# Runki2018/litehandnet

Measured on AMD Instinct MI355X. Metric: images/sec fwd+bwd @256x256 bs64 litehandnet, higher is better.
Workload: dtype f32; 1 GPU; litehandnet variant B (MSRB hourglass litehourglass.py) C=128, 256x256x3 -> 21x64x64, per-GPU batch 64, train-mode BN, fwd + TopdownHeatmapLoss + bwd + fused Adam; global_batch=64, parallelism=dp1

## Files before the change

### litehandnet_amd/csrc/k_conv_dw.hip

```cpp
#include <stdlib.h>
#include "lhn_common.h"

template <int K>
__global__ void __launch_bounds__(256) k_dw_fwd(lhn_view x, const float* __restrict__ w, lhn_view y,
                                                double* __restrict__ stats, int stride, int pad, int dil, lhn_bnfin fin,
                                                int ) {
  extern __shared__ __attribute__((aligned(16))) float smem[];
  const int C = x.C, C4 = C >> 2;
  constexpr int KK = K * K;
  float* Ws = smem;
  f4* red = reinterpret_cast<f4*>(smem + KK * C);
  const int tid = threadIdx.x;
  const int c4 = tid % C4, pl = tid / C4, PL = 256 / C4;
  const int cin = x.coff + 4 * c4, cout = y.coff + 4 * c4;
  const Xf4 xf = lhn_load_xf(x, cin);
  for (int i = tid; i < KK * C; i += 256) {
    const int c = i / KK, t = i - c * KK;
    Ws[t * C + c] = w ? w[i] : 1.f;
  }
  __syncthreads();
  f4 wt[KK];
#pragma unroll
  for (int t = 0; t < KK; ++t) wt[t] = *reinterpret_cast<const f4*>(Ws + t * C + 4 * c4);
  const int rows = y.N * y.H;
// ... 1309 lines not shown
            *reinterpret_cast<f4*>(o) = accx;
          }
        }
      }
    } else {
      if (dx)
        for (int j = 0; j < TH / 2; ++j) {
          const int rr = 2 * j + rpar, hh = th * TH + rr;
          if (wcol < SW && hh < SH && cok) {
            const int centre = ((rr + T::P) * T::WW + colw + T::P) * 8 + c4;
            f4 accx = (f4){0.f, 0.f, 0.f, 0.f};
            for (int a = 0; a < K; ++a)
#pragma unroll
              for (int b = 0; b < K; ++b)
                accx += tdy[centre - ((a * DIL - T::P) * T::WW + (b * DIL - T::P)) * 8] * wl[(a * K + b) * 8 + c4];
            float* o = dx + ((size_t)(n * x.H + pa + ps * hh) * x.W + pb + ps * wcol) * x.cstride + cx;
            if (dx_acc) accx += *reinterpret_cast<const f4*>(o);
            if (bs.add[0]) accx += *reinterpret_cast<const f4*>(bs.add[0] + (o - dx));
            if (bs.add[1]) accx += *reinterpret_cast<const f4*>(bs.add[1] + (o - dx));
            *reinterpret_cast<f4*>(o) = accx;
          }
        }
      for (int a = 0; a < K; ++a) {
        f4 ar[K];
#pragma unroll
        for (int b = 0; b < K; ++b) ar[b] = (f4){0.f, 0.f, 0.f, 0.f};
        for (int j = 0; j < TH / 2; ++j) {
          const int rr = 2 * j + rpar, hh = th * TH + rr;
          if (wcol < SW && hh < SH) {
            const int centre = ((rr + T::P) * T::WW + colw + T::P) * 8 + c4;
            const f4 dyc = tdy[centre];
#pragma unroll
            for (int b = 0; b < K; ++b) ar[b] += dyc * tx[centre + ((a * DIL - T::P) * T::WW + (b * DIL - T::P)) * 8];
          }
        }
#pragma unroll
        for (int b = 0; b < K; ++b) {
          f4 v = ar[b];
#pragma unroll
          for (int o = 8; o < 64; o <<= 1) {
            v.x += __shfl_xor(v.x, o, 64);
            v.y += __shfl_xor(v.y, o, 64);
            v.z += __shfl_xor(v.z, o, 64);
            v.w += __shfl_xor(v.w, o, 64);
          }
          if ((tid & 63) < 8) red[(tid >> 6) * 8 + c4 + 32 * b] = v;
        }
        __syncthreads();
        if (tid < 8 * K) {
          const int b = tid >> 3, cc = tid & 7;
          dws[(a * K + b) * 8 + cc] += red[cc + 32 * b] + red[8 + cc + 32 * b] + red[16 + cc + 32 * b] + red[24 + cc + 32 * b];
        }
        __syncthreads();
      }
    }
  }
  if (BNS) {
    double* st = bs.sums + (size_t)((bid / cgroups) % LHN_STAT_REPLICAS) * 2 * bs.C + bs.coff + cg * 32;
    lhn_block_stat_atomics(sdu, sdux, 8, red, st, st + bs.C);
  }
  float* dwr = dw + (size_t)((bid / cgroups) % nrep) * rep_stride;
  if (REGACC) {
#pragma unroll
    for (int k = 0; k < KK; ++k)
#pragma unroll
      for (int o = 8; o < 64; o <<= 1) {
        accw[k].x += __shfl_xor(accw[k].x, o, 64);
        accw[k].y += __shfl_xor(accw[k].y, o, 64);
        accw[k].z += __shfl_xor(accw[k].z, o, 64);
        accw[k].w += __shfl_xor(accw[k].w, o, 64);
      }
    __syncthreads();
    if ((tid & 63) < 8)
#pragma unroll
      for (int k = 0; k < KK; ++k) tdy[(k * 4 + (tid >> 6)) * 8 + c4] = accw[k];
    __syncthreads();
    if (tid < KK * 8) {
      const int k = tid >> 3, cc = tid & 7;
      const f4 sacc = tdy[(k * 4 + 0) * 8 + cc] + tdy[(k * 4 + 1) * 8 + cc] + tdy[(k * 4 + 2) * 8 + cc] + tdy[(k * 4 + 3) * 8 + cc];
      const int cb = cg * 32 + 4 * cc;
      if (cc < cvalid) {
        atomicAdd(dwr + (cb + 0) * KK + k, sacc.x);
        atomicAdd(dwr + (cb + 1) * KK + k, sacc.y);
        atomicAdd(dwr + (cb + 2) * KK + k, sacc.z);
        atomicAdd(dwr + (cb + 3) * KK + k, sacc.w);
      }
    }
  } else {
    __syncthreads();
    for (int i = tid; i < KK * 8; i += 256) {
      const int k = i >> 3, cb = cg * 32 + 4 * (i & 7);
      const f4 v = dws[i];
      if ((i & 7) >= cvalid) continue;
      atomicAdd(dwr + (cb + 0) * KK + k, v.x);
      atomicAdd(dwr + (cb + 1) * KK + k, v.y);
      atomicAdd(dwr + (cb + 2) * KK + k, v.z);
      atomicAdd(dwr + (cb + 3) * KK + k, v.w);
    }
  }
}

template <int DIL, bool BNS = false>
__global__ void __launch_bounds__(256, (BNS || DIL > 1) ? 2 : 3) k_dw3_bwd_rows(lhn_view x, const float* __restrict__ w, lhn_view y, lhn_gradview gy,
                                                         float* __restrict__ dx, int dx_acc, float* __restrict__ dw, int nstrips,
                                                         int nchunks, int CH, int cgroups, int nrep, int64_t rep_stride, int ps,
                                                         DwBnSum bs, lhn_bnbwdsrc fs) {
  constexpr int P = DIL, R = 2 * P + 2, WW = 32 + 2 * P, KK = 9;
  extern __shared__ __attribute__((aligned(16))) float smem[];
  f4* tdy = reinterpret_cast<f4*>(smem);
  f4* tx = tdy + R * WW * 8;
  f4* wl = tx + R * WW * 8;
  f4* cst = wl + KK * 8;
  f4* tmi = cst + KK * 8;
  f4* traw = tmi + 16;
  const int tid = threadIdx.x, c4 = tid & 7, pl = tid >> 3;
  const int ntile = y.N * ps * ps * nchunks * nstrips * cgroups;
  const int cg = blockIdx.x % cgroups;
  const int cvalid = min(8, (x.C - cg * 32) >> 2);
  const bool cok = c4 < cvalid;
  const int c4e = cok ? c4 : 0;
  const int cx = x.coff + cg * 32 + 4 * c4e, cy = y.coff + cg * 32 + 4 * c4e;
  const bool edge = tid < 16 * P;
  const int ecol = (pl < P) ? pl : 32 + pl;
  const f4 z = (f4){0.f, 0.f, 0.f, 0.f}, one = (f4){1.f, 1.f, 1.f, 1.f};
  if (tid < KK * 8) {
    const int k = tid >> 3, cc = cg * 32 + 4 * min(tid & 7, cvalid - 1);
    wl[tid] = (f4){w[(cc + 0) * KK + k], w[(cc + 1) * KK + k], w[(cc + 2) * KK + k], w[(cc + 3) * KK + k]};
  } else if (tid < 2 * KK * 8) {
    const int i = tid - KK * 8, kind = i >> 3, ca = cg * 32 + 4 * min(i & 7, cvalid - 1), j = kind % 3;
    const float* tab = kind < 3 ? x.table : kind < 6 ? y.table : gy.coef;
    const int cs = kind < 3 ? x.cstride : y.cstride, co = kind < 3 ? x.coff : y.coff;
    if (kind < 6 || !fs.sums) cst[i] = tab ? *reinterpret_cast<const f4*>(tab + j * cs + co + ca) : ((kind < 6 ? j != 1 : j == 0) ? one : z);
  } else if (BNS && tid < 2 * KK * 8 + 16) {
    const int i = tid - 2 * KK * 8, kind = i >> 3, cc = i & 7;
    tmi[i] = *reinterpret_cast<const f4*>(bs.save + kind * bs.C + bs.coff + cg * 32 + 4 * cc);
  }
  f4 accw[KK];
#pragma unroll
  for (int k = 0; k < KK; ++k) accw[k] = z;
  f4 sdu = z, sdux = z;
  struct Item {
    int n, pa, pb, SH, SW, wb, h0, nrows;
  };
  auto decode = [&](int t) __attribute__((always_inline)) {
    Item it;
    int r = t / cgroups;
    const int st = r % nstrips;
    r /= nstrips;
    const int ch = r % nchunks;
    r /= nchunks;
    const int par = r % (ps * ps);
    it.n = r / (ps * ps);
    it.pa = par / ps;
    it.pb = par % ps;
    it.SH = (x.H - it.pa + ps - 1) / ps;
    it.SW = (x.W - it.pb + ps - 1) / ps;
    it.wb = st * 32;
    it.h0 = ch * CH;
    it.nrows = max(0, min(CH, it.SH - it.h0));
    return it;
  };
  f4 mx = z, my = z, mz = z, mp = z, ex = z, ey = z, ez = z, ep = z;
  bool okm = false, oke = false;
  auto issue = [&](const Item& it, int hr) __attribute__((always_inline)) {
    const bool rok = hr >= 0 && hr < it.SH && cok;
    const int ih = it.pa + ps * hr;
    const int cm = it.wb + pl, ce = it.wb - P + ecol;
    okm = rok && cm < it.SW;
    oke = rok && edge && ce >= 0 && ce < it.SW;
    mx = my = mz = mp = ex = ey = ez = ep = z;
    if (okm) {
      const size_t pix = (size_t)(it.n * x.H + ih) * x.W + it.pb + ps * cm;
      mx = *reinterpret_cast<const f4*>(x.data + pix * x.cstride + cx);
      my = *reinterpret_cast<const f4*>(y.data + pix * y.cstride + cy);
      mz = *reinterpret_cast<const f4*>(gy.dz + pix * y.cstride + cy);
      if (gy.dpool) mp = lhn_dpool_sum(gy, y, it.n, ih, it.pb + ps * cm, cy);
    }
    if (oke) {
      const size_t pix = (size_t)(it.n * x.H + ih) * x.W + it.pb + ps * ce;
      ex = *reinterpret_cast<const f4*>(x.data + pix * x.cstride + cx);
      ey = *reinterpret_cast<const f4*>(y.data + pix * y.cstride + cy);
      ez = *reinterpret_cast<const f4*>(gy.dz + pix * y.cstride + cy);
      if (gy.dpool) ep = lhn_dpool_sum(gy, y, it.n, ih, it.pb + ps * ce, cy);
    }
  };
  auto put = [&](int s, int col, bool ok, f4 rx, f4 ry, f4 rz, f4 rp, f4 xg, f4 yg) __attribute__((always_inline)) {
    const f4 xsc = cst[c4], xsh = cst[8 + c4], xsl = cst[16 + c4];
    const f4 ysc = cst[24 + c4], ysh = cst[32 + c4], ysl = cst[40 + c4];
    const f4 gA = cst[48 + c4], gB = cst[56 + c4], gC = cst[64 + c4];
    const f4 ux = rx * xsc + xsh;
    const f4 vx = (f4){lhn_lrelu(ux.x, xsl.x), lhn_lrelu(ux.y, xsl.y), lhn_lrelu(ux.z, xsl.z), lhn_lrelu(ux.w, xsl.w)} * xg;
    const f4 e = rz * yg + rp;
    const f4 u = ry * ysc + ysh;
    const f4 dl = (f4){u.x > 0.f ? 1.f : ysl.x, u.y > 0.f ? 1.f : ysl.y, u.z > 0.f ? 1.f : ysl.z, u.w > 0.f ? 1.f : ysl.w};
    const f4 vy = gA * (e * dl) + gB * ry + gC;
    tx[(s * WW + col) * 8 + c4] = ok ? vx : z;
    tdy[(s * WW + col) * 8 + c4] = ok ? vy : z;
    if (BNS && col >= P && col < 32 + P) traw[(s * 32 + col - P) * 8 + c4] = rx;
  };
  int t = blockIdx.x;
  if (t < ntile) {
    const Item nx = decode(t);
    issue(nx, nx.h0 - P);
  }
  if (fs.sums) {
    float* cfA = reinterpret_cast<float*>(cst + 6 * 8);
    if (tid >= 4 * cvalid && tid < 32) cfA[tid] = cfA[32 + tid] = cfA[64 + tid] = 0.f;
    double* raw = reinterpret_cast<double*>(tdy);
    const int nc = 4 * cvalid;
    const LhnBwdPre pre = lhn_bn_bwd_pre(fs, cg * 32, nc);
    lhn_bn_bwd_fold_raw(fs.sums, fs.stat_channels, cg * 32, nc, raw);
    __syncthreads();
    if (tid < nc)
      lhn_bn_bwd_coef_put(lhn_bn_bwd_coef_raw(raw, nc, lhn_fin_groups(y.C), tid, pre, fs.count), fs, const_cast<float*>(gy.coef), y.cstride,
                          y.coff, cg * 32 + tid, cfA, 32, tid, (int)blockIdx.x < cgroups);
  }
#pragma unroll 1
  for (; t < ntile; t += gridDim.x) {
    const Item it = decode(t);
    const f4 xg = x.gate ? *reinterpret_cast<const f4*>(x.gate + (size_t)it.n * x.cstride + cx) : one;
    const f4 yg = y.gate ? *reinterpret_cast<const f4*>(y.gate + (size_t)it.n * y.cstride + cy) : one;
    const int wcol = it.wb + pl, nload = it.nrows + 2 * P;
    const bool ocol = wcol < it.SW;
    __syncthreads();
#pragma unroll 1
    for (int q = 0; q < nload; ++q) {
      const bool orow = q >= 2 * P;
      const int hh = it.h0 + max(q - 2 * P, 0);
      float* o = dx + ((size_t)(it.n * x.H + it.pa + ps * hh) * x.W + it.pb + ps * wcol) * x.cstride + cx;
      const bool st = orow && dx && cok && ocol;
      const int s = q % R;
      put(s, pl + P, okm, mx, my, mz, mp, xg, yg);
      if (edge) put(s, ecol, oke, ex, ey, ez, ep, xg, yg);
      if (q + 1 < nload) issue(it, it.h0 - P + q + 1);
      else if (t + (int)gridDim.x < ntile) {
        const Item nx = decode(t + gridDim.x);
        issue(nx, nx.h0 - P);
      }
      __syncthreads();
      if (!orow || !ocol) continue;
      int sr[3];
#pragma unroll
      for (int a = 0; a < 3; ++a) sr[a] = (q - 2 * P + a * DIL) % R;
      const int centre = (sr[1] * WW + pl + P) * 8 + c4;
      const f4 dyc = tdy[centre];
      f4 accx = z;
#pragma unroll
      for (int a = 0; a < 3; ++a) {
#pragma unroll
        for (int b = 0; b < 3; ++b) {
          accx += tdy[(sr[2 - a] * WW + pl + 2 * P - b * DIL) * 8 + c4] * wl[(a * 3 + b) * 8 + c4];
          accw[a * 3 + b] += dyc * tx[(sr[a] * WW + pl + b * DIL) * 8 + c4];
        }
      }
      if (BNS) {
        const f4 raw = traw[(sr[1] * 32 + pl) * 8 + c4];
        const f4 xsc = cst[c4], xsh = cst[8 + c4], xsl = cst[16 + c4];
        const f4 u = raw * xsc + xsh;
        const f4 du = accx * (f4){u.x > 0.f ? 1.f : xsl.x, u.y > 0.f ? 1.f : xsl.y, u.z > 0.f ? 1.f : xsl.z, u.w > 0.f ? 1.f : xsl.w};
        sdu += du;
        sdux += du * ((raw - tmi[c4]) * tmi[8 + c4]);
      }
      if (st) {
        if (dx_acc) accx += *reinterpret_cast<const f4*>(o);
        if (bs.add[0]) accx += *reinterpret_cast<const f4*>(bs.add[0] + (o - dx));
        if (bs.add[1]) accx += *reinterpret_cast<const f4*>(bs.add[1] + (o - dx));
        *reinterpret_cast<f4*>(o) = accx;
      }
    }
  }
  f4* red = tdy;
  if (BNS) {
    double* sts = bs.sums + (size_t)((blockIdx.x / cgroups) % LHN_STAT_REPLICAS) * 2 * bs.C + bs.coff + cg * 32;
    lhn_block_stat_atomics(sdu, sdux, 8, red, sts, sts + bs.C);
  }
  float* dwr = dw + (size_t)((blockIdx.x / cgroups) % nrep) * rep_stride;
#pragma unroll
  for (int k = 0; k < KK; ++k)
#pragma unroll
    for (int o = 8; o < 64; o <<= 1) {
      accw[k].x += __shfl_xor(accw[k].x, o, 64);
      accw[k].y += __shfl_xor(accw[k].y, o, 64);
      accw[k].z += __shfl_xor(accw[k].z, o, 64);
      accw[k].w += __shfl_xor(accw[k].w, o, 64);
    }
  __syncthreads();
  if ((tid & 63) < 8)
#pragma unroll
    for (int k = 0; k < KK; ++k) red[(k * 4 + (tid >> 6)) * 8 + c4] = accw[k];
  __syncthreads();
  if (tid < KK * 8) {
    const int k = tid >> 3, cc = tid & 7;
    const f4 sacc = red[(k * 4 + 0) * 8 + cc] + red[(k * 4 + 1) * 8 + cc] + red[(k * 4 + 2) * 8 + cc] + red[(k * 4 + 3) * 8 + cc];
    const int cb = cg * 32 + 4 * cc;
    if (cc < cvalid) {
      atomicAdd(dwr + (cb + 0) * KK + k, sacc.x);
      atomicAdd(dwr + (cb + 1) * KK + k, sacc.y);
      atomicAdd(dwr + (cb + 2) * KK + k, sacc.z);
      atomicAdd(dwr + (cb + 3) * KK + k, sacc.w);
    }
  }
}

static int dw3_xchunk(int grid, int cgroups) {
  static int on = -1;
  if (on < 0) {
    const char* e = getenv("LHN_XCD_ORDER");
    on = (e && e[0] == '1') ? 1 : 0;
  }
  return (on && grid % (8 * cgroups) == 0) ? grid / 8 : 0;
}
static int dw3_grid(int ntile, int cgroups, int per_cu) {
  int g = lhn_num_cus() * per_cu;
  g -= g % cgroups;
  if (g > ntile) g = ntile;
  if (g < cgroups) g = cgroups;
  return g;
}

template <int K, int DIL, int NS = 1>
static void launch_dwk_fwd(const lhn_view* x, const float* w, const lhn_view* y, double* stats, lhn_bnfin fin, hipStream_t s, int ps = 1,
                           const DwExtra* exp = nullptr) {
  DwExtra ex;
  if (exp) ex = *exp; else { ex.n = 0; ex.sum_out = nullptr; }
  constexpr int TH = 8, TW = 32, P = DIL * (K - 1) / 2;
  const int cg = (x->C + 31) / 32;
  const int sh = (y->H + ps - 1) / ps, sw = (y->W + ps - 1) / ps;
  const int th = (sh + TH - 1) / TH, tw = (sw + TW - 1) / TW, ntile = y->N * ps * ps * th * tw * cg;
  const size_t lds = (size_t)((TH + 2 * P) * (TW + 2 * P) * 8 + 512 + K * K * 8) * 16;
  const int per_cu = lds > 80 * 1024 ? 1 : (lds > 52 * 1024 ? 2 : 3);
  static LhnKernelCfg cfg;
  (void)lhn_kernel_cfg(cfg, &k_dwk_fwd_lds<K, DIL, NS>, lds, 4, nullptr);
  const int grid = dw3_grid(ntile, cg, per_cu * 2);
  hipLaunchKernelGGL((k_dwk_fwd_lds<K, DIL, NS>), dim3(grid), dim3(256), lds, s, *x, w, *y, stats, th, tw, cg, fin, ps, ex, dw3_xchunk(grid, cg));
}
template <int K, int DIL, bool BNS = false>
static void launch_dwk_bwd(const lhn_view* x, const float* w, const lhn_view* y, const lhn_gradview* gy, float* dx, int dx_acc,
                           float* dw, int nrep, int64_t rep_stride, hipStream_t s, int ps = 1, const DwBnSum* bsp = nullptr) {
  constexpr int TH = 8, TW = 16, P = DIL * (K - 1) / 2;
  DwBnSum bs;
  if (bsp) bs = *bsp; else { bs.sums = nullptr; bs.save = nullptr; bs.C = bs.coff = 0; bs.add[0] = bs.add[1] = nullptr; }
  const int cg = (x->C + 31) / 32;
  const int sh = (x->H + ps - 1) / ps, sw = (x->W + ps - 1) / ps;
  const int th = (sh + TH - 1) / TH, tw = (sw + TW - 1) / TW, ntile = x->N * ps * ps * th * tw * cg;
  const size_t lds = (size_t)((TH + 2 * P) * (TW + 2 * P) * 16 + 256 + 2 * K * K * 8 + (BNS ? TH * TW * 8 + 16 : 0)) * 16;
  static LhnKernelCfg cfg;
  (void)lhn_kernel_cfg(cfg, &k_dwk_bwd_lds<K, DIL, BNS>, lds, 4, nullptr);
  const int grid = dw3_grid(ntile, cg, 4);
  hipLaunchKernelGGL((k_dwk_bwd_lds<K, DIL, BNS>), dim3(grid), dim3(256), lds, s, *x, w, *y, *gy, dx, dx_acc, dw, th, tw,
                     cg, nrep, rep_stride, ps, bs, dw3_xchunk(grid, cg));
}
template <int DIL, bool BNS = false>
static void launch_dw3_bwd_rows(const lhn_view* x, const float* w, const lhn_view* y, const lhn_gradview* gy, float* dx, int dx_acc,
                                float* dw, int nrep, int64_t rep_stride, hipStream_t s, int ps = 1, const DwBnSum* bsp = nullptr,
                                const lhn_bnbwdsrc* fsp = nullptr) {
  constexpr int P = DIL, R = 2 * P + 2, WW = 32 + 2 * P;
  DwBnSum bs;
  if (bsp) bs = *bsp; else { bs.sums = nullptr; bs.save = nullptr; bs.C = bs.coff = 0; bs.add[0] = bs.add[1] = nullptr; }
  lhn_bnbwdsrc fs;
  if (fsp) fs = *fsp; else memset(&fs, 0, sizeof(fs));
  static_assert(R * WW * 8 * 16 >= 2 * LHN_FIN_THREADS * 8, "dy ring holds the replica fold's partials");
  const int cg = (x->C + 31) / 32;
  const int sh = (x->H + ps - 1) / ps, sw = (x->W + ps - 1) / ps;
  const int nstrips = (sw + 31) / 32;
  const size_t lds = (size_t)(2 * R * WW * 8 + 2 * 9 * 8 + 16 + (BNS ? R * 32 * 8 : 0)) * 16;
  static LhnKernelCfg cfg;
  int per_cu = 1;
  (void)lhn_kernel_cfg(cfg, &k_dw3_bwd_rows<DIL, BNS>, lds, 8, &per_cu);
  const int base = x->N * ps * ps * nstrips * cg;
  int nch = (lhn_num_cus() * per_cu + base - 1) / base;
  nch = std::max(1, std::min(nch, (sh + 7) / 8));
  const int CH = (sh + nch - 1) / nch;
  nch = (sh + CH - 1) / CH;
  const int ntile = base * nch;
  const int grid = dw3_grid(ntile, cg, per_cu);
  hipLaunchKernelGGL((k_dw3_bwd_rows<DIL, BNS>), dim3(grid), dim3(256), lds, s, *x, w, *y, *gy, dx, dx_acc, dw, nstrips, nch, CH, cg,
                     nrep, rep_stride, ps, bs, fs);
}
static bool lhn_dw_bwd_v1() {
  static int v = -1;
  if (v < 0) {
    const char* e = getenv("LHN_DW_BWD_V1");
    v = (e && e[0] == '1') ? 1 : 0;
  }
  return v == 1;
}


struct DwS2 {
  static constexpr int TH = 4, TW = 16, XH = 2 * TH + 1, XW = 2 * TW + 1, XPIX = XH * XW, DH = TH + 1, DW = TW + 1, DPIX = DH * DW;
};

__global__ void __launch_bounds__(256) k_dws2_fwd_lds(lhn_view x, const float* __restrict__ w, lhn_view y, double* __restrict__ stats,
                                                      int tiles_h, int tiles_w, int cgroups, lhn_bnfin fin) {
  using T = DwS2;
  extern __shared__ __attribute__((aligned(16))) float smem[];
  f4* tx = reinterpret_cast<f4*>(smem);
  f4* red = tx + T::XPIX * 8;
  f4* wl = red + 512;
  const int tid = threadIdx.x, c4 = tid & 7, pl = tid >> 3;
  const int ntile = y.N * tiles_h * tiles_w * cgroups;
  const int cg = blockIdx.x % cgroups;
  const int cvalid = min(8, (x.C - cg * 32) >> 2);
  const bool cok = c4 < cvalid;
  const int c4e = cok ? c4 : 0;
  const int cin = x.coff + cg * 32 + 4 * c4e, cout = y.coff + cg * 32 + 4 * c4e;
  for (int i = tid; i < 72; i += 256) {
    const int k = i >> 3, cc = cg * 32 + 4 * min(i & 7, cvalid - 1);
    wl[i] = (f4){w[(cc + 0) * 9 + k], w[(cc + 1) * 9 + k], w[(cc + 2) * 9 + k], w[(cc + 3) * 9 + k]};
  }
  const Xf4 xf = lhn_load_xf(x, cin);
  double sd[4] = {0, 0, 0, 0}, qd[4] = {0, 0, 0, 0};
  constexpr int NIT = (T::XPIX + 31) / 32;
  for (int t = blockIdx.x; t < ntile; t += gridDim.x) {
    int r = t / cgroups;
    const int tw = r % tiles_w;
    r /= tiles_w;
    const int th = r % tiles_h, n = r / tiles_h;
    const int h0 = 2 * th * T::TH - 1, w0 = 2 * tw * T::TW - 1;
    const f4 gate = x.gate ? *reinterpret_cast<const f4*>(x.gate + (size_t)n * x.cstride + cin) : (f4){1.f, 1.f, 1.f, 1.f};
    const float* xin = x.data + (size_t)n * x.H * x.W * x.cstride + cin;
    f4 raw[NIT];
#pragma unroll
    for (int it = 0; it < NIT; ++it) {
      const int i = min(pl + 32 * it, T::XPIX - 1);
      const int ph = i / T::XW, pw = i - ph * T::XW;
      const int ih = min(max(h0 + ph, 0), x.H - 1), iw = min(max(w0 + pw, 0), x.W - 1);
      raw[it] = *reinterpret_cast<const f4*>(xin + ((size_t)ih * x.W + iw) * x.cstride);
    }
    __syncthreads();
#pragma unroll
    for (int it = 0; it < NIT; ++it) {
      const int i = pl + 32 * it;
      if (i < T::XPIX) {
        const int ph = i / T::XW, pw = i - ph * T::XW;
        const int ih = h0 + ph, iw = w0 + pw;
        const bool inb = ih >= 0 && ih < x.H && iw >= 0 && iw < x.W;
        tx[i * 8 + c4] = inb ? lhn_apply_xf(raw[it], xf) * gate : (f4){0.f, 0.f, 0.f, 0.f};
      }
    }
    __syncthreads();
    f4 s = (f4){0.f, 0.f, 0.f, 0.f}, q = s, kk = s;
    int cnt = 0;
#pragma unroll
    for (int j = 0; j < 2; ++j) {
      const int o = pl + 32 * j, oh = o / T::TW, ow = o - oh * T::TW;
      const int ho = th * T::TH + oh, wo = tw * T::TW + ow;
      if (cok && ho < y.H && wo < y.W) {
        f4 acc = (f4){0.f, 0.f, 0.f, 0.f};
#pragma unroll
        for (int a = 0; a < 3; ++a)
#pragma unroll
          for (int b = 0; b < 3; ++b) acc += tx[((2 * oh + a) * T::XW + 2 * ow + b) * 8 + c4] * wl[(a * 3 + b) * 8 + c4];
        *reinterpret_cast<f4*>(y.data + ((size_t)(n * y.H + ho) * y.W + wo) * y.cstride + cout) = acc;
        if (cnt == 0) kk = acc;
        const f4 d = acc - kk;
        s += d;
        q += d * d;
        ++cnt;
      }
    }
    lhn_unshift4(sd, qd, s, q, kk, cnt);
  }
  if (stats) {
    const int C = x.C;
    double* st = stats + (size_t)((blockIdx.x / cgroups) % LHN_STAT_REPLICAS) * 2 * C + cg * 32;
    lhn_block_stat_atomics_d(sd, qd, 8, reinterpret_cast<double*>(red), st, st + C, cvalid);
    if (fin.counter && lhn_last_block(fin.counter)) lhn_bn_finalize_block(fin, stats);
  }
}

__global__ void __launch_bounds__(256, 2) k_dws2_bwd_lds(lhn_view x, const float* __restrict__ w, lhn_view y, lhn_gradview gy,
                                                      float* __restrict__ dx, int dx_acc, float* __restrict__ dw, int tiles_h,
                                                      int tiles_w, int cgroups, int nrep, int64_t rep_stride) {
  using T = DwS2;
  extern __shared__ __attribute__((aligned(16))) float smem[];
  f4* tx = reinterpret_cast<f4*>(smem);
  f4* tdy = tx + T::XPIX * 8;
  f4* wl = tdy + T::DPIX * 8;
  const int tid = threadIdx.x, c4 = tid & 7, pl = tid >> 3;
  const int ntile = y.N * tiles_h * tiles_w * cgroups;
  const int cg = blockIdx.x % cgroups;
  const int cvalid = min(8, (x.C - cg * 32) >> 2);
  const bool cok = c4 < cvalid;
  const int c4e = cok ? c4 : 0;
  const int cx = x.coff + cg * 32 + 4 * c4e, cy = y.coff + cg * 32 + 4 * c4e;
  const Xf4 xxf = lhn_load_xf(x, cx), yxf = lhn_load_xf(y, cy);
  const Gr4 ygr = lhn_load_coef(gy, y.cstride, cy);
  for (int i = tid; i < 72; i += 256) {
    const int k = i >> 3, cc = cg * 32 + 4 * min(i & 7, cvalid - 1);
    wl[i] = (f4){w[(cc + 0) * 9 + k], w[(cc + 1) * 9 + k], w[(cc + 2) * 9 + k], w[(cc + 3) * 9 + k]};
  }
  f4 accw[9];
#pragma unroll
  for (int k = 0; k < 9; ++k) accw[k] = (f4){0.f, 0.f, 0.f, 0.f};
  constexpr int NITX = (T::XPIX + 31) / 32, NITD = (T::DPIX + 31) / 32;
  for (int t = blockIdx.x; t < ntile; t += gridDim.x) {
    int r = t / cgroups;
    const int tw = r % tiles_w;
    r /= tiles_w;
    const int th = r % tiles_h, n = r / tiles_h;
    const int h0 = 2 * th * T::TH - 1, w0 = 2 * tw * T::TW - 1;
    const int oh0 = th * T::TH, ow0 = tw * T::TW;
    const f4 xgate = x.gate ? *reinterpret_cast<const f4*>(x.gate + (size_t)n * x.cstride + cx) : (f4){1.f, 1.f, 1.f, 1.f};
    f4 rx[NITX], ry[NITD], rz[NITD];
#pragma unroll
    for (int it = 0; it < NITX; ++it) {
      const int i = min(pl + 32 * it, T::XPIX - 1);
      const int ph = i / T::XW, pw = i - ph * T::XW;
      const int ih = min(max(h0 + ph, 0), x.H - 1), iw = min(max(w0 + pw, 0), x.W - 1);
      rx[it] = *reinterpret_cast<const f4*>(x.data + ((size_t)(n * x.H + ih) * x.W + iw) * x.cstride + cx);
    }
#pragma unroll
    for (int it = 0; it < NITD; ++it) {
      const int i = min(pl + 32 * it, T::DPIX - 1);
      const int ph = i / T::DW, pw = i - ph * T::DW;
      const int ho = min(oh0 + ph, y.H - 1), wo = min(ow0 + pw, y.W - 1);
      const size_t off = ((size_t)(n * y.H + ho) * y.W + wo) * y.cstride + cy;
      ry[it] = *reinterpret_cast<const f4*>(y.data + off);
      rz[it] = *reinterpret_cast<const f4*>(gy.dz + off);
    }
    __syncthreads();
#pragma unroll
    for (int it = 0; it < NITX; ++it) {
      const int i = pl + 32 * it;
      if (i < T::XPIX) {
        const int ph = i / T::XW, pw = i - ph * T::XW;
        const int ih = h0 + ph, iw = w0 + pw;
        const bool inb = ih >= 0 && ih < x.H && iw >= 0 && iw < x.W;
        tx[i * 8 + c4] = inb ? lhn_apply_xf(rx[it], xxf) * xgate : (f4){0.f, 0.f, 0.f, 0.f};
      }
    }
#pragma unroll
    for (int it = 0; it < NITD; ++it) {
      const int i = pl + 32 * it;
      if (i < T::DPIX) {
        const int ph = i / T::DW, pw = i - ph * T::DW;
        const int ho = oh0 + ph, wo = ow0 + pw;
        f4 d = (f4){0.f, 0.f, 0.f, 0.f};
        if (ho < y.H && wo < y.W) {
          const f4 du = lhn_grad_du(y, gy, yxf, ry[it], rz[it], n, ho, wo, cy);
          d = ygr.A * du + ygr.B * ry[it] + ygr.Cc;
        }
        tdy[i * 8 + c4] = d;
      }
    }
    __syncthreads();
#pragma unroll
    for (int j = 0; j < 2; ++j) {
      const int o = pl + 32 * j, oh = o / T::TW, ow = o - oh * T::TW;
      const f4 dyc = tdy[(oh * T::DW + ow) * 8 + c4];
#pragma unroll
      for (int a = 0; a < 3; ++a)
#pragma unroll
        for (int b = 0; b < 3; ++b) accw[a * 3 + b] += dyc * tx[((2 * oh + a) * T::XW + 2 * ow + b) * 8 + c4];
    }
    if (dx && cok) {
      const int c = pl, iw = 2 * ow0 + c;
      const int nb = (c & 1) ? 2 : 1;
      const int bA = (c & 1) ? 0 : 1, colA = (c & 1) ? (c + 1) >> 1 : c >> 1, colB = (c - 1) >> 1;
      if (iw < x.W) {
#pragma unroll
        for (int rr = 0; rr < 2 * T::TH; ++rr) {
          const int ih = 2 * oh0 + rr;
          if (ih < x.H) {
            f4 accx = (f4){0.f, 0.f, 0.f, 0.f};
            if ((rr & 1) == 0) {
              const f4* drow = tdy + ((rr >> 1) * T::DW) * 8 + c4;
              accx += drow[colA * 8] * wl[(3 + bA) * 8 + c4];
              if (nb == 2) accx += drow[colB * 8] * wl[(3 + 2) * 8 + c4];
            } else {
              const f4* d0 = tdy + (((rr + 1) >> 1) * T::DW) * 8 + c4;
              const f4* d2 = tdy + (((rr - 1) >> 1) * T::DW) * 8 + c4;
              accx += d0[colA * 8] * wl[(0 + bA) * 8 + c4] + d2[colA * 8] * wl[(6 + bA) * 8 + c4];
              if (nb == 2) accx += d0[colB * 8] * wl[(0 + 2) * 8 + c4] + d2[colB * 8] * wl[(6 + 2) * 8 + c4];
            }
            float* o = dx + ((size_t)(n * x.H + ih) * x.W + iw) * x.cstride + cx;
            if (dx_acc) accx += *reinterpret_cast<const f4*>(o);
            *reinterpret_cast<f4*>(o) = accx;
          }
        }
      }
    }
  }
  float* dwr = dw + (size_t)((blockIdx.x / cgroups) % nrep) * rep_stride;
#pragma unroll
  for (int k = 0; k < 9; ++k)
#pragma unroll
    for (int o = 8; o < 64; o <<= 1) {
      accw[k].x += __shfl_xor(accw[k].x, o, 64);
      accw[k].y += __shfl_xor(accw[k].y, o, 64);
      accw[k].z += __shfl_xor(accw[k].z, o, 64);
      accw[k].w += __shfl_xor(accw[k].w, o, 64);
    }
  __syncthreads();
  if ((tid & 63) < 8)
#pragma unroll
    for (int k = 0; k < 9; ++k) tdy[(k * 4 + (tid >> 6)) * 8 + c4] = accw[k];
  __syncthreads();
  if (tid < 72) {
    const int k = tid >> 3, cc = tid & 7;
    const f4 sacc = tdy[(k * 4 + 0) * 8 + cc] + tdy[(k * 4 + 1) * 8 + cc] + tdy[(k * 4 + 2) * 8 + cc] + tdy[(k * 4 + 3) * 8 + cc];
    const int cb = cg * 32 + 4 * cc;
    if (cc < cvalid) {
      atomicAdd(dwr + (cb + 0) * 9 + k, sacc.x);
      atomicAdd(dwr + (cb + 1) * 9 + k, sacc.y);
      atomicAdd(dwr + (cb + 2) * 9 + k, sacc.z);
      atomicAdd(dwr + (cb + 3) * 9 + k, sacc.w);
    }
  }
}

static int dws2_fwd(const lhn_view* x, const float* w, const lhn_view* y, double* stats, lhn_bnfin fin, hipStream_t s) {
  using T = DwS2;
  const int cg = (x->C + 31) / 32;
  const int th = (y->H + T::TH - 1) / T::TH, tw = (y->W + T::TW - 1) / T::TW, ntile = y->N * th * tw * cg;
  size_t lds = (size_t)(T::XPIX * 8 + 512 + 72) * 16;
  static LhnKernelCfg cfg;
  if (!lhn_kernel_cfg(cfg, &k_dws2_fwd_lds, lds, 4, nullptr)) return 0;
  hipLaunchKernelGGL(k_dws2_fwd_lds, dim3(dw3_grid(ntile, cg, 6)), dim3(256), lds, s, *x, w, *y, stats, th, tw, cg, fin);
  return 1;
}
static int dws2_bwd(const lhn_view* x, const float* w, const lhn_view* y, const lhn_gradview* gy, float* dx, int dx_acc, float* dw,
                    int nrep, int64_t rep_stride, hipStream_t s) {
  using T = DwS2;
  const int cg = (x->C + 31) / 32;
  const int th = (y->H + T::TH - 1) / T::TH, tw = (y->W + T::TW - 1) / T::TW, ntile = y->N * th * tw * cg;
  const size_t lds = (size_t)((T::XPIX + T::DPIX) * 8 + 72) * 16;
  static LhnKernelCfg cfg;
  if (!lhn_kernel_cfg(cfg, &k_dws2_bwd_lds, lds, 4, nullptr)) return 0;
  hipLaunchKernelGGL(k_dws2_bwd_lds, dim3(dw3_grid(ntile, cg, 4)), dim3(256), lds, s, *x, w, *y, *gy, dx, dx_acc, dw, th, tw, cg, nrep, rep_stride);
  return 1;
}

int lhn_dwk_fwd_lds(const lhn_view* x, const float* w, const lhn_view* y, double* stats, int k, int dil, lhn_bnfin fin,
                    hipStream_t s, const DwExtra* ex) {
  if (ex && ex->n > 0) {
    if (k == 3 && dil == 1) launch_dwk_fwd<3, 1, 2>(x, w, y, stats, fin, s, 1, ex);
    else if (k == 3 && dil == 2 && y->W >= 16) launch_dwk_fwd<3, 1, 2>(x, w, y, stats, fin, s, 2, ex);
    else return 0;
    return 1;
  }
  if (k == 3 && dil == 1) launch_dwk_fwd<3, 1>(x, w, y, stats, fin, s, 1, ex);
  else if (k == 3 && dil == 2 && y->W >= 16) launch_dwk_fwd<3, 1>(x, w, y, stats, fin, s, 2, ex);
  else if (k == 3 && dil == 2) launch_dwk_fwd<3, 2>(x, w, y, stats, fin, s, 1, ex);
  else if (k == 7 && dil == 1) launch_dwk_fwd<7, 1>(x, w, y, stats, fin, s, 1, ex);
  else return 0;
  return 1;
}
int lhn_dwk_bwd_lds(const lhn_view* x, const float* w, const lhn_view* y, const lhn_gradview* gy, float* dx, int dx_acc,
                    float* dw, int k, int dil, int nrep, int64_t rep_stride, hipStream_t s, const DwBnSum* bs,
                    const lhn_bnbwdsrc* fs) {
  if (fs && (lhn_dw_bwd_v1() || k != 3)) return 0;
  if (bs && bs->sums) {
    if (!(k == 3 && dil == 1 && dx && !dx_acc)) return 0;
    if (lhn_dw_bwd_v1()) launch_dwk_bwd<3, 1, true>(x, w, y, gy, dx, dx_acc, dw, nrep, rep_stride, s, 1, bs);
    else launch_dw3_bwd_rows<1, true>(x, w, y, gy, dx, dx_acc, dw, nrep, rep_stride, s, 1, bs, fs);
    return 1;
  }
  const bool v1 = lhn_dw_bwd_v1();
  if (k == 3 && dil == 1) {
    if (v1) launch_dwk_bwd<3, 1>(x, w, y, gy, dx, dx_acc, dw, nrep, rep_stride, s, 1, bs);
    else launch_dw3_bwd_rows<1>(x, w, y, gy, dx, dx_acc, dw, nrep, rep_stride, s, 1, bs, fs);
  } else if (k == 3 && dil == 2 && x->W >= 16) {
    if (v1) launch_dwk_bwd<3, 1>(x, w, y, gy, dx, dx_acc, dw, nrep, rep_stride, s, 2, bs);
    else launch_dw3_bwd_rows<1>(x, w, y, gy, dx, dx_acc, dw, nrep, rep_stride, s, 2, bs, fs);
  } else if (k == 3 && dil == 2) {
    if (v1) launch_dwk_bwd<3, 2>(x, w, y, gy, dx, dx_acc, dw, nrep, rep_stride, s, 1, bs);
    else launch_dw3_bwd_rows<2>(x, w, y, gy, dx, dx_acc, dw, nrep, rep_stride, s, 1, bs, fs);
  } else if (k == 7 && dil == 1) launch_dwk_bwd<7, 1>(x, w, y, gy, dx, dx_acc, dw, nrep, rep_stride, s, 1, bs);
  else return 0;
  return 1;
}

static int dw_fwd_extra(const lhn_view* x, const float* w, const lhn_view* y, double* stats, int k, int stride, int pad, int dil,
                        lhn_bnfin fin, const lhn_view* extra, const float* coef, const lhn_view* so, hipStream_t s) {
  if (!(stride == 1 && pad == dil * (k - 1) / 2 && x->C % 4 == 0 && y->W >= 8)) return 0;
  if (!lhn_no_pend(x) || !lhn_no_pend(extra)) return 0;
  DwExtra ex;
  ex.v = *extra;
  ex.coef[0] = coef[0];
  ex.coef[1] = coef[1];
  ex.n = 1;
  ex.sum_out = so ? so->data : nullptr;
  ex.so_cstride = so ? so->cstride : 0;
  ex.so_coff = so ? so->coff : 0;
  return lhn_dwk_fwd_lds(x, w, y, stats, k, dil, fin, s, &ex);
}

static int dw_bwd_addends(const lhn_view* x, const float* w, const lhn_view* y, const lhn_gradview* gy, float* dx, int dx_acc, float* dw,
                          int k, int dil, int nrep, int64_t rep_stride, const float* a0, const float* a1, hipStream_t s) {
  DwBnSum bs;
  bs.sums = nullptr;
  bs.save = nullptr;
  bs.C = bs.coff = 0;
  bs.add[0] = a0;
  bs.add[1] = a1;
  return lhn_dwk_bwd_lds(x, w, y, gy, dx, dx_acc, dw, k, dil, nrep, rep_stride, s, &bs);
}

static int dw_bwd_fin(const lhn_view* x, const float* w, const lhn_view* y, const lhn_gradview* gy, float* dx, int dx_acc, float* dw, int k,
                      int dil, int nrep, int64_t rep_stride, const lhn_bnsum* bns, const float* a0, const float* a1, const lhn_bnbwdsrc* fin,
                      hipStream_t s) {
  DwBnSum bs;
  bs.sums = bns ? bns->sums : nullptr;
  bs.save = bns ? bns->save : nullptr;
  bs.C = bns ? bns->C : 0;
  bs.coff = bns ? bns->coff : 0;
  bs.add[0] = a0;
  bs.add[1] = a1;
  return lhn_dwk_bwd_lds(x, w, y, gy, dx, dx_acc, dw, k, dil, nrep, rep_stride, s, &bs, fin);
}

static int dw_bwd_fused(const lhn_view* x, const float* w, const lhn_view* y, const lhn_gradview* gy, float* dx, float* dw, int k,
                        int dil, int nrep, int64_t rep_stride, double* bn_sums, const float* bn_save, int bn_C, int bn_coff, hipStream_t s) {
  DwBnSum bs;
  bs.sums = bn_sums;
  bs.save = bn_save;
  bs.C = bn_C;
  bs.coff = bn_coff;
  bs.add[0] = bs.add[1] = nullptr;
  return lhn_dwk_bwd_lds(x, w, y, gy, dx, 0, dw, k, dil, nrep, rep_stride, s, &bs);
}
```

Measured before the change: 8994 images/s.

## Add 8x8 spatial-tile depthwise 3x3 backward kernel for small feature maps

Adds a new depthwise 3x3 backward kernel that works on 8x8 output tiles with a one-pixel halo in LDS. It prefetches the next tile's x, y and dy into registers while computing the current one, and accumulates the weight gradient per block with shuffle reduction and atomics. A dispatcher sends small feature maps (up to 32x32, with few total tiles) to this kernel instead of the row-strip kernel. The aim is to give small layers more parallelism than row strips can. The cost is more halo loads per tile and more dw atomics.

Measured after the change: 9037 images/s (median of 6 runs). Within noise of the previous version (+0.5%).

```diff
diff --git a/litehandnet_amd/csrc/k_conv_dw.hip b/litehandnet_amd/csrc/k_conv_dw.hip
--- a/litehandnet_amd/csrc/k_conv_dw.hip
+++ b/litehandnet_amd/csrc/k_conv_dw.hip
@@ -1635,6 +1635,206 @@
   }
 }
 
+template <bool BNS = false>
+__global__ void __launch_bounds__(256, 2) k_dw3_bwd_tile(lhn_view x, const float* __restrict__ w, lhn_view y, lhn_gradview gy,
+                                                         float* __restrict__ dx, int dx_acc, float* __restrict__ dw, int tiles_h,
+                                                         int tiles_w, int cgroups, int nrep, int64_t rep_stride, int ps, DwBnSum bs,
+                                                         lhn_bnbwdsrc fs) {
+  constexpr int TH = 8, TW = 8, WW = TW + 2, PIX = (TH + 2) * WW, KK = 9, NIT = (PIX + 31) / 32;
+  constexpr int RP = 32 / TW, NJ = TH / RP;
+  static_assert(2 * PIX * 8 * 16 >= 2 * LHN_FIN_THREADS * 8, "the two tiles hold the replica fold's partials");
+  extern __shared__ __attribute__((aligned(16))) float smem[];
+  f4* tdy = reinterpret_cast<f4*>(smem);
+  f4* tx = tdy + PIX * 8;
+  f4* wl = tx + PIX * 8;
+  f4* cst = wl + KK * 8;
+  f4* tmi = cst + KK * 8;
+  f4* traw = tmi + 16;
+  const int tid = threadIdx.x, c4 = tid & 7, pl = tid >> 3;
+  const int colw = pl % TW, rpar = pl / TW;
+  const int ntile = y.N * ps * ps * tiles_h * tiles_w * cgroups;
+  const int cg = blockIdx.x % cgroups;
+  const int cvalid = min(8, (x.C - cg * 32) >> 2);
+  const bool cok = c4 < cvalid;
+  const int c4e = cok ? c4 : 0;
+  const int cx = x.coff + cg * 32 + 4 * c4e, cy = y.coff + cg * 32 + 4 * c4e;
+  const f4 z = (f4){0.f, 0.f, 0.f, 0.f}, one = (f4){1.f, 1.f, 1.f, 1.f};
+  f4 accw[KK];
+#pragma unroll
+  for (int k = 0; k < KK; ++k) accw[k] = z;
+  f4 sdu = z, sdux = z;
+  struct Item {
+    int n, pa, pb, SH, SW, th, tw;
+  };
+  auto decode = [&](int t) __attribute__((always_inline)) {
+    Item it;
+    int r = t / cgroups;
+    it.tw = r % tiles_w;
+    r /= tiles_w;
+    it.th = r % tiles_h;
+    r /= tiles_h;
+    const int par = r % (ps * ps);
+    it.n = r / (ps * ps);
+    it.pa = par / ps;
+    it.pb = par % ps;
+    it.SH = (x.H - it.pa + ps - 1) / ps;
+    it.SW = (x.W - it.pb + ps - 1) / ps;
+    return it;
+  };
+  f4 rx[NIT], ry[NIT], rz[NIT], rp[NIT], xg = one, yg = one;
+#pragma unroll
+  for (int q = 0; q < NIT; ++q) rp[q] = z;
+  auto issue = [&](const Item& it) __attribute__((always_inline)) {
+    const int h0 = it.th * TH - 1, w0 = it.tw * TW - 1;
+    const size_t img = (size_t)it.n * x.H * x.W;
+    const float* xb = x.data + img * x.cstride;
+    const float* yb = y.data + img * y.cstride;
+    const float* zb = gy.dz + img * y.cstride;
+#pragma unroll
+    for (int q = 0; q < NIT; ++q) {
+      const int i = min(pl + 32 * q, PIX - 1);
+      const int ph = i / WW, pw = i - ph * WW;
+      const int ih = min(it.pa + ps * min(max(h0 + ph, 0), max(it.SH - 1, 0)), x.H - 1);
+      const int iw = min(it.pb + ps * min(max(w0 + pw, 0), max(it.SW - 1, 0)), x.W - 1);
+      const unsigned pix = (unsigned)(ih * x.W + iw);
+      rx[q] = *reinterpret_cast<const f4*>(xb + (pix * (unsigned)x.cstride + (unsigned)cx));
+      ry[q] = *reinterpret_cast<const f4*>(yb + (pix * (unsigned)y.cstride + (unsigned)cy));
+      rz[q] = *reinterpret_cast<const f4*>(zb + (pix * (unsigned)y.cstride + (unsigned)cy));
+      if (gy.dpool) rp[q] = lhn_dpool_sum(gy, y, it.n, ih, iw, cy);
+    }
+    if (x.gate) xg = *reinterpret_cast<const f4*>(x.gate + (size_t)it.n * x.cstride + cx);
+    if (y.gate) yg = *reinterpret_cast<const f4*>(y.gate + (size_t)it.n * y.cstride + cy);
+  };
+  auto commit = [&](const Item& it) __attribute__((always_inline)) {
+    const int h0 = it.th * TH - 1, w0 = it.tw * TW - 1;
+    const f4 xsc = cst[c4], xsh = cst[8 + c4], xsl = cst[16 + c4];
+    const f4 ysc = cst[24 + c4], ysh = cst[32 + c4], ysl = cst[40 + c4];
+    const f4 gA = cst[48 + c4], gB = cst[56 + c4], gC = cst[64 + c4];
+#pragma unroll
+    for (int q = 0; q < NIT; ++q) {
+      const int i = pl + 32 * q;
+      if (i < PIX) {
+        const int ph = i / WW, pw = i - ph * WW;
+        const int hh = h0 + ph, ww = w0 + pw;
+        const bool inb = hh >= 0 && hh < it.SH && ww >= 0 && ww < it.SW;
+        const f4 ux = rx[q] * xsc + xsh;
+        const f4 vx = (f4){lhn_lrelu(ux.x, xsl.x), lhn_lrelu(ux.y, xsl.y), lhn_lrelu(ux.z, xsl.z), lhn_lrelu(ux.w, xsl.w)} * xg;
+        const f4 e = rz[q] * yg + rp[q];
+        const f4 u = ry[q] * ysc + ysh;
+        const f4 dl = (f4){u.x > 0.f ? 1.f : ysl.x, u.y > 0.f ? 1.f : ysl.y, u.z > 0.f ? 1.f : ysl.z, u.w > 0.f ? 1.f : ysl.w};
+        const f4 vy = gA * (e * dl) + gB * ry[q] + gC;
+        tx[i * 8 + c4] = inb ? vx : z;
+        tdy[i * 8 + c4] = inb ? vy : z;
+        if (BNS && ph >= 1 && ph <= TH && pw >= 1 && pw <= TW) traw[((ph - 1) * TW + pw - 1) * 8 + c4] = rx[q];
+      }
+    }
+  };
+  int t = blockIdx.x;
+  if (t < ntile) issue(decode(t));
+  if (tid < KK * 8) {
+    const int k = tid >> 3, cc = cg * 32 + 4 * min(tid & 7, cvalid - 1);
+    wl[tid] = (f4){w[(cc + 0) * KK + k], w[(cc + 1) * KK + k], w[(cc + 2) * KK + k], w[(cc + 3) * KK + k]};
+  } else if (tid < 2 * KK * 8) {
+    const int i = tid - KK * 8, kind = i >> 3, ca = cg * 32 + 4 * min(i & 7, cvalid - 1), j = kind % 3;
+    const float* tab = kind < 3 ? x.table : kind < 6 ? y.table : gy.coef;
+    const int cs = kind < 3 ? x.cstride : y.cstride, co = kind < 3 ? x.coff : y.coff;
+    if (kind < 6 || !fs.sums) cst[i] = tab ? *reinterpret_cast<const f4*>(tab + j * cs + co + ca) : ((kind < 6 ? j != 1 : j == 0) ? one : z);
+  } else if (BNS && tid < 2 * KK * 8 + 16) {
+    const int i = tid - 2 * KK * 8, kind = i >> 3, cc = i & 7;
+    tmi[i] = *reinterpret_cast<const f4*>(bs.save + kind * bs.C + bs.coff + cg * 32 + 4 * cc);
+  }
+  if (fs.sums) {
+    float* cfA = reinterpret_cast<float*>(cst + 6 * 8);
+    if (tid >= 4 * cvalid && tid < 32) cfA[tid] = cfA[32 + tid] = cfA[64 + tid] = 0.f;
+    double* raw = reinterpret_cast<double*>(tdy);
+    const int nc = 4 * cvalid;
+    const LhnBwdPre pre = lhn_bn_bwd_pre(fs, cg * 32, nc);
+    lhn_bn_bwd_fold_raw(fs.sums, fs.stat_channels, cg * 32, nc, raw);
+    __syncthreads();
+    if (tid < nc)
+      lhn_bn_bwd_coef_put(lhn_bn_bwd_coef_raw(raw, nc, lhn_fin_groups(y.C), tid, pre, fs.count), fs, const_cast<float*>(gy.coef), y.cstride,
+                          y.coff, cg * 32 + tid, cfA, 32, tid, (int)blockIdx.x < cgroups);
+  }
+#pragma unroll 1
+  for (; t < ntile; t += gridDim.x) {
+    const Item it = decode(t);
+    const int wcol = it.tw * TW + colw;
+    __syncthreads();
+    commit(it);
+    f4 ad[NJ];
+#pragma unroll
+    for (int j = 0; j < NJ; ++j) {
+      const int hh = it.th * TH + j * RP + rpar;
+      ad[j] = z;
+      if (!BNS && wcol < it.SW && hh < it.SH && dx && cok) {
+        const size_t o = ((size_t)(it.n * x.H + it.pa + ps * hh) * x.W + it.pb + ps * wcol) * x.cstride + cx;
+        if (dx_acc) ad[j] = *reinterpret_cast<const f4*>(dx + o);
+        if (bs.add[0]) ad[j] += *reinterpret_cast<const f4*>(bs.add[0] + o);
+        if (bs.add[1]) ad[j] += *reinterpret_cast<const f4*>(bs.add[1] + o);
+      }
+    }
+    __syncthreads();
+#pragma unroll
+    for (int j = 0; j < NJ; ++j) {
+      const int rr = j * RP + rpar, hh = it.th * TH + rr;
+      if (!(wcol < it.SW && hh < it.SH)) continue;
+      const int centre = ((rr + 1) * WW + colw + 1) * 8 + c4;
+      const f4 dyc = tdy[centre];
+      f4 accx = z;
+#pragma unroll
+      for (int a = 0; a < 3; ++a)
+#pragma unroll
+        for (int b = 0; b < 3; ++b) {
+          const int off = ((a - 1) * WW + (b - 1)) * 8;
+          accx += tdy[centre - off] * wl[(a * 3 + b) * 8 + c4];
+          accw[a * 3 + b] += dyc * tx[centre + off];
+        }
+      if (BNS) {
+        const f4 raw = traw[(rr * TW + colw) * 8 + c4];
+        const f4 xsc = cst[c4], xsh = cst[8 + c4], xsl = cst[16 + c4];
+        const f4 u = raw * xsc + xsh;
+        const f4 du = accx * (f4){u.x > 0.f ? 1.f : xsl.x, u.y > 0.f ? 1.f : xsl.y, u.z > 0.f ? 1.f : xsl.z, u.w > 0.f ? 1.f : xsl.w};
+        sdu += du;
+        sdux += du * ((raw - tmi[c4]) * tmi[8 + c4]);
+      }
+      if (!BNS) accx += ad[j];
+      if (dx && cok) *reinterpret_cast<f4*>(dx + ((size_t)(it.n * x.H + it.pa + ps * hh) * x.W + it.pb + ps * wcol) * x.cstride + cx) = accx;
+    }
+    if (t + (int)gridDim.x < ntile) issue(decode(t + gridDim.x));
+  }
+  f4* red = tdy;
+  if (BNS) {
+    double* sts = bs.sums + (size_t)((blockIdx.x / cgroups) % LHN_STAT_REPLICAS) * 2 * bs.C + bs.coff + cg * 32;
+    lhn_block_stat_atomics(sdu, sdux, 8, red, sts, sts + bs.C);
+  }
+  float* dwr = dw + (size_t)((blockIdx.x / cgroups) % nrep) * rep_stride;
+#pragma unroll
+  for (int k = 0; k < KK; ++k)
+#pragma unroll
+    for (int o = 8; o < 64; o <<= 1) {
+      accw[k].x += __shfl_xor(accw[k].x, o, 64);
+      accw[k].y += __shfl_xor(accw[k].y, o, 64);
+      accw[k].z += __shfl_xor(accw[k].z, o, 64);
+      accw[k].w += __shfl_xor(accw[k].w, o, 64);
+    }
+  __syncthreads();
+  if ((tid & 63) < 8)
+#pragma unroll
+    for (int k = 0; k < KK; ++k) red[(k * 4 + (tid >> 6)) * 8 + c4] = accw[k];
+  __syncthreads();
+  if (tid < KK * 8) {
+    const int k = tid >> 3, cc = tid & 7;
+    const f4 sacc = red[(k * 4 + 0) * 8 + cc] + red[(k * 4 + 1) * 8 + cc] + red[(k * 4 + 2) * 8 + cc] + red[(k * 4 + 3) * 8 + cc];
+    const int cb = cg * 32 + 4 * cc;
+    if (cc < cvalid) {
+      atomicAdd(dwr + (cb + 0) * KK + k, sacc.x);
+      atomicAdd(dwr + (cb + 1) * KK + k, sacc.y);
+      atomicAdd(dwr + (cb + 2) * KK + k, sacc.z);
+      atomicAdd(dwr + (cb + 3) * KK + k, sacc.w);
+    }
+  }
+}
+
 static int dw3_xchunk(int grid, int cgroups) {
   static int on = -1;
   if (on < 0) {
@@ -1710,6 +1910,41 @@
   hipLaunchKernelGGL((k_dw3_bwd_rows<DIL, BNS>), dim3(grid), dim3(256), lds, s, *x, w, *y, *gy, dx, dx_acc, dw, nstrips, nch, CH, cg,
                      nrep, rep_stride, ps, bs, fs);
 }
+template <bool BNS = false>
+static void launch_dw3_bwd_tile(const lhn_view* x, const float* w, const lhn_view* y, const lhn_gradview* gy, float* dx, int dx_acc,
+                                float* dw, int nrep, int64_t rep_stride, hipStream_t s, int ps, const DwBnSum* bsp, const lhn_bnbwdsrc* fsp) {
+  constexpr int TH = 8, TW = 8, PIX = (TH + 2) * (TW + 2);
+  DwBnSum bs;
+  if (bsp) bs = *bsp; else { bs.sums = nullptr; bs.save = nullptr; bs.C = bs.coff = 0; bs.add[0] = bs.add[1] = nullptr; }
+  lhn_bnbwdsrc fs;
+  if (fsp) fs = *fsp; else memset(&fs, 0, sizeof(fs));
+  const int cg = (x->C + 31) / 32;
+  const int sh = (x->H + ps - 1) / ps, sw = (x->W + ps - 1) / ps;
+  const int th = (sh + TH - 1) / TH, tw = (sw + TW - 1) / TW, ntile = x->N * ps * ps * th * tw * cg;
+  const size_t lds = (size_t)(2 * PIX * 8 + 2 * 9 * 8 + 16 + (BNS ? TH * TW * 8 : 0)) * 16;
+  static LhnKernelCfg cfg;
+  int per_cu = 1;
+  (void)lhn_kernel_cfg(cfg, &k_dw3_bwd_tile<BNS>, lds, 8, &per_cu);
+  const int grid = dw3_grid(ntile, cg, per_cu);
+  hipLaunchKernelGGL((k_dw3_bwd_tile<BNS>), dim3(grid), dim3(256), lds, s, *x, w, *y, *gy, dx, dx_acc, dw, th, tw, cg, nrep,
+                     rep_stride, ps, bs, fs);
+}
+static bool dw3_small_tile(int sh, int sw, int C, int nimg) {
+  static int on = -1;
+  if (on < 0) {
+    const char* e = getenv("LHN_DW_BWD_SMALL");
+    on = (e && e[0] == '0') ? 0 : 1;
+  }
+  if (!on || sh > 32 || sw > 32) return false;
+  return (int64_t)nimg * ((C + 31) / 32) * ((sh + 7) / 8) * ((sw + 7) / 8) <= 512;
+}
+template <bool BNS>
+static void launch_dw3_bwd_s1(const lhn_view* x, const float* w, const lhn_view* y, const lhn_gradview* gy, float* dx, int dx_acc, float* dw,
+                              int nrep, int64_t rep_stride, hipStream_t s, int ps, const DwBnSum* bs, const lhn_bnbwdsrc* fs) {
+  if (dw3_small_tile((x->H + ps - 1) / ps, (x->W + ps - 1) / ps, x->C, x->N * ps * ps))
+    launch_dw3_bwd_tile<BNS>(x, w, y, gy, dx, dx_acc, dw, nrep, rep_stride, s, ps, bs, fs);
+  else launch_dw3_bwd_rows<1, BNS>(x, w, y, gy, dx, dx_acc, dw, nrep, rep_stride, s, ps, bs, fs);
+}
 static bool lhn_dw_bwd_v1() {
   static int v = -1;
   if (v < 0) {
@@ -1988,16 +2223,16 @@
   if (bs && bs->sums) {
     if (!(k == 3 && dil == 1 && dx && !dx_acc)) return 0;
     if (lhn_dw_bwd_v1()) launch_dwk_bwd<3, 1, true>(x, w, y, gy, dx, dx_acc, dw, nrep, rep_stride, s, 1, bs);
-    else launch_dw3_bwd_rows<1, true>(x, w, y, gy, dx, dx_acc, dw, nrep, rep_stride, s, 1, bs, fs);
+    else launch_dw3_bwd_s1<true>(x, w, y, gy, dx, dx_acc, dw, nrep, rep_stride, s, 1, bs, fs);
     return 1;
   }
   const bool v1 = lhn_dw_bwd_v1();
   if (k == 3 && dil == 1) {
     if (v1) launch_dwk_bwd<3, 1>(x, w, y, gy, dx, dx_acc, dw, nrep, rep_stride, s, 1, bs);
-    else launch_dw3_bwd_rows<1>(x, w, y, gy, dx, dx_acc, dw, nrep, rep_stride, s, 1, bs, fs);
+    else launch_dw3_bwd_s1<false>(x, w, y, gy, dx, dx_acc, dw, nrep, rep_stride, s, 1, bs, fs);
   } else if (k == 3 && dil == 2 && x->W >= 16) {
     if (v1) launch_dwk_bwd<3, 1>(x, w, y, gy, dx, dx_acc, dw, nrep, rep_stride, s, 2, bs);
-    else launch_dw3_bwd_rows<1>(x, w, y, gy, dx, dx_acc, dw, nrep, rep_stride, s, 2, bs, fs);
+    else launch_dw3_bwd_s1<false>(x, w, y, gy, dx, dx_acc, dw, nrep, rep_stride, s, 2, bs, fs);
   } else if (k == 3 && dil == 2) {
     if (v1) launch_dwk_bwd<3, 2>(x, w, y, gy, dx, dx_acc, dw, nrep, rep_stride, s, 1, bs);
     else launch_dw3_bwd_rows<2>(x, w, y, gy, dx, dx_acc, dw, nrep, rep_stride, s, 1, bs, fs);
```
